# paperwave/STIF-continuous-video-representation

Measured on AMD Instinct MI355X. Metric: upsampled Mpix/sec at 7×128×128→4× scale, 1/2/4/8 MI355X; PSNR vs ref, higher is better.
Workload: dtype f16x3; 1 GPU; per GPU 7x3x128x128 window (6 pairs), 4.0x spatial, t=[0.5]; frames=7, parallelism=1 GPU

## Files before the change

stif-continuous-video-representation_amd/csrc/decoder.hip:

```cpp
#include "dec_layout.h"
#include "stif_common.h"
#include "tuning.h"
#include "stif.h"
#include "abi_util.h"

#include <algorithm>
#include <climits>
#include <cstdio>
#include <type_traits>

namespace {

using namespace stif_dec;

template <int F16>
struct XT;
template <>
struct XT<0> {
  f32x16 v;
};
template <>
struct XT<1> {
  f16x8 h[2], l[2];
};
// ... 73 lines not shown
  b.w00 = (vx0 && vy0) ? wx0 * wy0 : 0.f;
  b.w01 = (vx1 && vy0) ? wx1 * wy0 : 0.f;
  b.w10 = (vx0 && vy1) ? wx0 * wy1 : 0.f;
  b.w11 = (vx1 && vy1) ? wx1 * wy1 : 0.f;
  return b;
}
STIF_DEV Bilin bilin(float gx, float gy, int Wd, int Hd) {
  const Corners c = bilin_corners(gx, gy, Wd, Hd);
  Bilin b;
  b.o00 = c.cy0 * Wd + c.cx0; b.o01 = c.cy0 * Wd + c.cx1; b.o10 = c.cy1 * Wd + c.cx0; b.o11 = c.cy1 * Wd + c.cx1;
  b.w00 = c.w00; b.w01 = c.w01; b.w10 = c.w10; b.w11 = c.w11;
  return b;
}

template <class TAB>
STIF_DEV Bilin bilin_tab(const TAB& tb, int py, int px, int pitch) {
  Bilin b;
  const int *by0 = tb.by0, *by1 = tb.by1, *bx0 = tb.bx0, *bx1 = tb.bx1;
  const float *wy0_ = tb.wy0, *wy1_ = tb.wy1, *wx0_ = tb.wx0, *wx1_ = tb.wx1;
  const int y0 = by0[py], y1 = by1[py], x0 = bx0[px], x1 = bx1[px];
  const float wy0 = wy0_[py], wy1 = wy1_[py], wx0 = wx0_[px], wx1 = wx1_[px];
  b.o00 = y0 * pitch + x0; b.o01 = y0 * pitch + x1; b.o10 = y1 * pitch + x0; b.o11 = y1 * pitch + x1;
  b.w00 = wx0 * wy0; b.w01 = wx1 * wy0; b.w10 = wx0 * wy1; b.w11 = wx1 * wy1;
  return b;
}

struct WarpGrids {
  float g1x, g1y, g2x, g2y;
};
STIF_DEV WarpGrids warp_grids(const f32x4 fv, float bx, float by, int WW, int HH) {
  const float lo = -1.f + 1e-6f, hi = 1.f - 1e-6f;
  const float dx = ((float)WW - 1.f) / 2.f, dy = ((float)HH - 1.f) / 2.f;
  WarpGrids g;
  g.g1x = fminf(fmaxf(bx + fv[0] / dx, lo), hi), g.g1y = fminf(fmaxf(by + fv[1] / dy, lo), hi);
  g.g2x = fminf(fmaxf(bx + fv[2] / dx, lo), hi), g.g2y = fminf(fmaxf(by + fv[3] / dy, lo), hi);
  return g;
}

constexpr int GRID = 0, WINDOW = 1, PTS = 2;

template <bool OR>
STIF_DEV void report_range_w(int* status, bool bad) {
  if constexpr (OR) {
    if (status != nullptr && bad) atomicOr(status, 1);
  } else {
    report_range(status, bad);
  }
}

template <int FORM>
STIF_DEV Bilin bilin_hr(float gx, float gy, int WW, int HH, const stif_dec_window& win, int* status, int slot = 0) {
  if constexpr (FORM == GRID) {
    return bilin(gx, gy, WW, HH);
  } else if constexpr (FORM == PTS) {
    const Corners c = bilin_corners(gx, gy, WW, HH);
    Bilin b;
    b.o00 = slot; b.o01 = slot + 1; b.o10 = slot + 2; b.o11 = slot + 3;
    b.w00 = c.w00; b.w01 = c.w01; b.w10 = c.w10; b.w11 = c.w11;
    return b;
  } else {
    const Corners c = bilin_corners(gx, gy, WW, HH);
    const int ry0 = c.cy0 - win.fy0, ry1 = c.cy1 - win.fy0, rx0 = c.cx0 - win.fx0, rx1 = c.cx1 - win.fx0;
    const int y0 = min(max(ry0, 0), win.fh - 1), y1 = min(max(ry1, 0), win.fh - 1);
    const int x0 = min(max(rx0, 0), win.fw - 1), x1 = min(max(rx1, 0), win.fw - 1);
    if (status != nullptr && (y0 != ry0 || y1 != ry1 || x0 != rx0 || x1 != rx1)) atomicOr(status, 2);
    Bilin b;
    b.o00 = y0 * win.fw + x0; b.o01 = y0 * win.fw + x1; b.o10 = y1 * win.fw + x0; b.o11 = y1 * win.fw + x1;
    b.w00 = c.w00; b.w01 = c.w01; b.w10 = c.w10; b.w11 = c.w11;
    return b;
  }
}

template <int GPB>
STIF_DEV void gather64(f32x16* dst, const float* __restrict__ base, int stride, int c0, const Bilin& b, int hf) {
  const int c = c0 + 4 * hf;
  const float* p00 = base + (size_t)b.o00 * stride + c;
  const float* p01 = base + (size_t)b.o01 * stride + c;
  const float* p10 = base + (size_t)b.o10 * stride + c;
  const float* p11 = base + (size_t)b.o11 * stride + c;
#pragma unroll
  for (int g0 = 0; g0 < 8; g0 += GPB) {
    f32x4 cr[GPB][4];
#pragma unroll
    for (int g = 0; g < GPB; ++g) {
      const int o = 8 * (g0 + g);
      cr[g][0] = ld4(p00 + o);
      cr[g][1] = ld4(p01 + o);
      cr[g][2] = ld4(p10 + o);
      cr[g][3] = ld4(p11 + o);
    }
#pragma unroll
    for (int g = 0; g < GPB; ++g) {
      f32x4 s = b.w00 * cr[g][0] + b.w01 * cr[g][1] + b.w10 * cr[g][2] + b.w11 * cr[g][3];
      asm volatile("" : "+v"(s));
      const int gg = g0 + g;
#pragma unroll
      for (int e = 0; e < 4; ++e) dst[gg >> 2][4 * (gg & 3) + e] = s[e];
    }
    if constexpr (GPB < 8) asm volatile("" ::: "memory");
  }
}

STIF_DEV void img_mma(f32x16* z, const float* __restrict__ wt, const f32x4 im4, int lane) {
#pragma unroll
  for (int ot = 0; ot < 2; ++ot) {
    const f32x4 w0 = ld4(wt + ot * T + lane * 4);
#pragma unroll
    for (int e = 0; e < 4; ++e) z[ot] = mfma32(w0[e], im4[e], z[ot]);
  }
}

STIF_DEV f32x4 img_sample(const float* __restrict__ I, const Bilin& b, int hf) {
  const float* c = I + 4 * hf;
  return b.w00 * ld4(c + b.o00 * IMG_C) + b.w01 * ld4(c + b.o01 * IMG_C) + b.w10 * ld4(c + b.o10 * IMG_C) +
         b.w11 * ld4(c + b.o11 * IMG_C);
}

struct Pixel {
  bool valid;
  long long pc;
  int item, ly, lx;
  int pt;
};
STIF_DEV void point_yx(const stif_dec_points& pts, int item, int pt, int HH, int WW, int* status, int& y, int& x) {
  const int ry = pts.y[item * pts.y_item + pt], rx = pts.x[item * pts.x_item + pt];
  y = min(max(ry, 0), HH - 1), x = min(max(rx, 0), WW - 1);
  if (status != nullptr && (y != ry || x != rx)) atomicOr(status, 8);
}
template <int NW, int PPW, int FORM, class TQ>
STIF_DEV Pixel pixel_of(int wv, int lane, int n, int HH, int WW, const stif_dec_window& win, const TQ& tq,
                        int* status) {
  Pixel o;
  if constexpr (FORM == PTS) {
    const long long total = (long long)n * tq.npts;
    const long long p = ((long long)xcd_block(blockIdx.x, gridDim.x) * NW + wv) * PPW + (lane & (PPW - 1));
    o.valid = p < total;
    o.pc = o.valid ? p : total - 1;
    o.item = (int)(o.pc / tq.npts);
    o.pt = (int)(o.pc - (long long)o.item * tq.npts);
    point_yx(tq, o.item, o.pt, HH, WW, status, o.ly, o.lx);
  } else {
    constexpr bool WIN = FORM == WINDOW;
    const int GH = WIN ? win.hh : HH, GW = WIN ? win.ww : WW;
    const long long total = (long long)n * GH * GW;
    const long long p = ((long long)xcd_block(blockIdx.x, gridDim.x) * NW + wv) * PPW + (lane & (PPW - 1));
    o.valid = p < total;
    o.pc = o.valid ? p : total - 1;
    o.item = (int)(o.pc / ((long long)GH * GW));
    const int rem = (int)(o.pc - (long long)o.item * GH * GW);
    o.ly = rem / GW, o.lx = rem - o.ly * GW;
    o.pt = 0;
  }
  return o;
}

template <int TQ>
struct TimeArg {
  typedef const float* __restrict__ type;
};
template <>
struct TimeArg<1> {
  typedef stif_dec_time type;
};
template <>
struct TimeArg<2> {
  typedef stif_dec_points type;
};
template <int FORM, bool TF>
constexpr int TQK = FORM == PTS ? 2 : TF ? 1 : 0;
template <int TQ>
STIF_DEV float time_at(const typename TimeArg<TQ>::type& tq, int item, int gy, int gx, int pt = 0) {
  if constexpr (TQ == 2) return tq.t[item * tq.t_item + pt * tq.t_point];
  else if constexpr (TQ == 1) return tq.t[item * tq.item + gy * tq.row + gx * tq.col];
  else return tq[item];
}

STIF_DEV float blend_weight(const stif_dec_blend& bl, int gy, int gx) {
#pragma clang fp contract(off)
  float a[4];
#pragma unroll
  for (int j = 0; j < 4; ++j) a[j] = __fadd_rn(fabsf(__fmul_rn(bl.rel_y[j][gy], bl.rel_x[j][gx])), 1e-9f);
  const float tot = __fadd_rn(__fadd_rn(__fadd_rn(a[0], a[1]), a[2]), a[3]);
  const float ak = bl.k == 0 ? a[3] : bl.k == 1 ? a[2] : bl.k == 2 ? a[1] : a[0];
  return __fdiv_rn(ak, tot);
}

template <int FORM, bool REPORT, bool BLEND = false>
STIF_DEV void store_rgb(float* __restrict__ out, const float* __restrict__ mlp, const float* o4, const f32x4 fv,
                        int item, int py, int px, int HH, int WW, const stif_dec_window& win, int* status,
                        const stif_dec_blend& bl) {
  constexpr bool WIN = FORM == WINDOW;
  static_assert(WIN || !BLEND, "the blending epilogue is the windowed stages'");
  const size_t plane = WIN ? (size_t)win.out_plane : (size_t)HH * WW;
  float* o = WIN ? out + (size_t)item * win.out_item + (size_t)py * win.out_pitch + px
                 : out + (size_t)item * 3 * plane + (size_t)py * WW + px;
  bool bad = not_finite((fv[0] + fv[1]) + (fv[2] + fv[3]));
  float rgb[3];
#pragma unroll
  for (int c = 0; c < 3; ++c) {
    rgb[c] = o4[c] + mlp[E_B4 + c];
    bad |= not_finite(rgb[c]);
    if constexpr (!BLEND) o[c * plane] = rgb[c];
  }
  if constexpr (BLEND) {
    const float wk = blend_weight(bl, win.y0 + py, win.x0 + px);
    if (!bl.accumulate) {
#pragma unroll
      for (int c = 0; c < 3; ++c) o[c * plane] = __fmul_rn(rgb[c], wk);
    } else {
#pragma unroll
      for (int c = 0; c < 3; ++c) o[c * plane] = __fmaf_rn(rgb[c], wk, o[c * plane]);
    }
  }
  if constexpr (REPORT) report_range_w<FORM != GRID>(status, bad);
}

constexpr int NW1 = 4;
constexpr int DEC2_NW = 4;
constexpr int DEC2_WPE = 2;
constexpr int SEG = 10;
constexpr int SEG1 = 8;

STIF_DEV void dec_dma(__amdgpu_buffer_rsrc_t rm, float* dst, int lane, int soff) {
  __builtin_amdgcn_raw_ptr_buffer_load_lds(rm, dst, 16, (unsigned)(lane * 16), soff, 0, 0);
}
template <int NW>
STIF_DEV void dma_tiles(float* dst, __amdgpu_buffer_rsrc_t rm, int src, int ntiles, int wv, int lane) {
  if ((ntiles * 4) % NW == 0) {
#pragma unroll
    for (int i = 0; i < ntiles * 4 / NW; ++i)
      dec_dma(rm, dst + (wv + i * NW) * 256, lane, (src + (wv + i * NW) * 256) * 4);
  } else {
    for (int k = wv; k < ntiles * 4; k += NW)
      dec_dma(rm, dst + k * 256, lane, (src + k * 256) * 4);
  }
}

STIF_DEV __amdgpu_buffer_rsrc_t mlp_rsrc(const float* mlp) {
  return __builtin_amdgcn_make_buffer_rsrc((void*)mlp, (short)0, (int)(MLP_FLOATS * 4), 0x00020000);
}

template <int F16>
STIF_DEV void tile_mma(f32x16& acc, const float* t, const XT<F16>& xt, int lane) {
  const float* b = t + lane * 4;
  if constexpr (F16) {
#pragma unroll
    for (int m = 0; m < 2; ++m) {
      const f16x8 ah = ldh8(b + (2 * m) * 256), al = ldh8(b + (2 * m + 1) * 256);
      acc = mfma16h(ah, xt.h[m], acc);
      acc = mfma16h(al, xt.h[m], acc);
      acc = mfma16h(ah, xt.l[m], acc);
    }
  } else {
    const f32x16& x = xt.v;
    const f32x4 w0 = ld4(b), w1 = ld4(b + 256), w2 = ld4(b + 512), w3 = ld4(b + 768);
#pragma unroll
    for (int e = 0; e < 4; ++e) acc = mfma32(w0[e], x[e], acc);
#pragma unroll
    for (int e = 0; e < 4; ++e) acc = mfma32(w1[e], x[4 + e], acc);
#pragma unroll
    for (int e = 0; e < 4; ++e) acc = mfma32(w2[e], x[8 + e], acc);
#pragma unroll
    for (int e = 0; e < 4; ++e) acc = mfma32(w3[e], x[12 + e], acc);
  }
  __builtin_amdgcn_sched_barrier(0);
}

template <int NO>
STIF_DEV void narrow_dot(float* o, const float* W, int kt, const f32x16& x, int hf) {
#pragma unroll
  for (int c = 0; c < NO; ++c)
#pragma unroll
    for (int v = 0; v < 4; ++v) {
      const f32x4 w = ld4(W + c * 256 + kt * 32 + 8 * v + 4 * hf);
#pragma unroll
      for (int e = 0; e < 4; ++e) o[c] = fmaf(w[e], x[4 * v + e], o[c]);
    }
}

template <int MODE, bool HRIMG>
constexpr int OCC1 = MODE == 2 ? 2 : HRIMG ? 3 : 4;
template <int MODE, bool HRIMG>
constexpr int S1 = OCC1<MODE, HRIMG> == 4 ? 4 : OCC1<MODE, HRIMG> == 3 ? 6 : SEG1;
template <int MODE, bool HRIMG, int F16, int FORM, bool TF = false>
__global__ __launch_bounds__(NW1 * 64) __attribute__((amdgpu_waves_per_eu(OCC1<MODE, HRIMG>))) void k_dec1(const float* __restrict__ proj, const float* __restrict__ mlp,
                                                     stif_dec_tables tb, stif_dec_image im,
                                                     typename TimeArg<TQK<FORM, TF>>::type tq, float* __restrict__ hrfeat,
                                                     float* __restrict__ flow, int n, int h, int w, int HH,
                                                     int WW, stif_dec_window win, int* status) {
  constexpr bool WIN = FORM == WINDOW;
  constexpr int TQ = TQK<FORM, TF>;
  static_assert(!(WIN && MODE == 2 && HRIMG), "the windowed flow-only stage takes no high-resolution image");
  static_assert(!TF || (MODE != 2 && !HRIMG), "a time field has no local-ensemble and no HR-image form");
  static_assert(FORM != PTS || (MODE != 2 && !HRIMG && !TF), "a point list has no local-ensemble and no HR-image form");
  constexpr bool OCC3 = S1<MODE, HRIMG> != SEG1;
  constexpr bool OCC4 = OCC1<MODE, HRIMG> == 4;
  __shared__ __attribute__((aligned(16))) float wbuf[2 * S1<MODE, HRIMG> * T + T];
  const int lane = threadIdx.x & 63, hf = lane >> 5;
  const int wv = __builtin_amdgcn_readfirstlane(threadIdx.x >> 6);
  float* const B0 = wbuf;
  float* const B1 = wbuf + S1<MODE, HRIMG> * T;
  float* const W3V = wbuf + 2 * S1<MODE, HRIMG> * T;
  const __amdgpu_buffer_rsrc_t rm = mlp_rsrc(mlp);
  if (MODE != 1) dma_tiles<NW1>(W3V, rm, L_W3V, 1, wv, lane);
  if (MODE != 2) dma_tiles<NW1>(B0, rm, F_W1, 4, wv, lane);
  else {
    dma_tiles<NW1>(B1, rm, L_W0, 4, wv, lane);
    dma_tiles<NW1>(B1 + 4 * T, rm, L_W1, 4, wv, lane);
  }
  const Pixel pix = pixel_of<NW1, 32, FORM>(wv, lane, n, HH, WW, win, tq, status);
  const bool valid = pix.valid;
  const long long pc = pix.pc;
  const int item = pix.item;
  const int py = WIN ? win.y0 + pix.ly : pix.ly, px = WIN ? win.x0 + pix.lx : pix.lx;
  const float t = TF ? 0.f : time_at<TQ>(tq, item, py, px, pix.pt);
  auto time = [&]() {
    if constexpr (TF) return time_at<TQ>(tq, item, py, px);
    else return t;
  };
  const float* P = proj + (size_t)item * h * w * PROJ_C;

  f32x16 hr[2] = {f32x16{0}, f32x16{0}};
  f32x16 x1[2];
  if constexpr (MODE != 2) {
  f32x16 x0[2];
  {
    const float ry = tb.rel_y[py], rx = tb.rel_x[px], t = time();
    const float* p1 = P + ((size_t)tb.near_y[py] * w + tb.near_x[px]) * PROJ_C;
#pragma unroll
    for (int ot = 0; ot < 2; ++ot)
#pragma unroll
      for (int v = 0; v < 4; ++v) {
        const int f = ot * 32 + 8 * v + 4 * hf;
        const f32x4 z = ld4(p1 + f) + ld4(mlp + F_WRY + f) * ry + ld4(mlp + F_WRX + f) * rx + ld4(mlp + F_WT + f) * t;
#pragma unroll
        for (int e = 0; e < 4; ++e) x0[ot][4 * v + e] = siren_sin<F16>(z[e]);
      }
  }
  auto seg_feat23 = [&](float* dst, int kt) {
#pragma unroll
    for (int r = 0; r < 16 / NW1; ++r) {
      const int i = wv + r * NW1, j = i >> 2;
      const int src = (j < 2 ? F_W2 + (kt * 2 + j) * T : F_W3 + ((j - 2) * 8 + kt) * T) + (i & 3) * 256;
      dec_dma(rm, dst + j * T + (i & 3) * 256, lane, src * 4);
    }
  };
  lds_dma_barrier();
  const Bias32 fb1[2] = {bias_ld(mlp + F_B1, hf), bias_ld(mlp + F_B1 + 32, hf)};
  __builtin_amdgcn_sched_barrier(0);
  seg_feat23(B1, 0);
  {
    const XT<F16> xs[2] = {xop<F16>(x0[0]), xop<F16>(x0[1])};
#pragma unroll
    for (int ot = 0; ot < 2; ++ot) {
      f32x16 acc = f32x16{0};
#pragma unroll
      for (int kt = 0; kt < 2; ++kt) tile_mma<F16>(acc, B0 + (ot * 2 + kt) * T, xs[kt], lane);
      x1[ot] = bias_sin<F16>(acc, fb1[ot]);
    }
  }
  const XT<F16> x1s[2] = {xop<F16>(x1[0]), xop<F16>(x1[1])};
  auto feat_step = [&](int kt, bool last) {
    lds_dma_barrier();
    const Bias32 b2 = bias_ld(mlp + F_B2 + kt * 32, hf);
    __builtin_amdgcn_sched_barrier(0);
    float* cur = (kt & 1) ? B0 : B1;
    float* nxt = (kt & 1) ? B1 : B0;
    if (!last) seg_feat23(nxt, kt + 1);
    else {
      dma_tiles<NW1>(nxt, rm, L_W0, 4, wv, lane);
      if (!OCC4) dma_tiles<NW1>(nxt + 4 * T, rm, L_W1, OCC3 ? 2 : 4, wv, lane);
    }
    f32x16 acc = f32x16{0};
    tile_mma<F16>(acc, cur, x1s[0], lane);
    tile_mma<F16>(acc, cur + T, x1s[1], lane);
    const XT<F16> h2 = xop<F16>(bias_sin<F16>(acc, b2));
    tile_mma<F16>(hr[0], cur + 2 * T, h2, lane);
    tile_mma<F16>(hr[1], cur + 3 * T, h2, lane);
  };
#pragma unroll 1
  for (int kt = 0; kt < 7; ++kt) feat_step(kt, false);
  feat_step(7, true);
#pragma unroll
  for (int ot = 0; ot < 2; ++ot) hr[ot] = bias_add<F16>(hr[ot], mlp + F_B3 + ot * 32, hf);
  if (valid) {
    float* o = hrfeat + (WIN ? ((size_t)item * win.fh + (py - win.fy0)) * win.fw + (px - win.fx0) : (size_t)pc) * 64;
#pragma unroll
    for (int ot = 0; ot < 2; ++ot)
#pragma unroll
      for (int v = 0; v < 4; ++v) {
        f32x4 s;
#pragma unroll
        for (int e = 0; e < 4; ++e) s[e] = hr[ot][4 * v + e];
        st4(o + ot * 32 + 8 * v + 4 * hf, s);
      }
  }
  }
  if constexpr (MODE == 1) return;
  if constexpr (MODE == 2) {
    Bilin b;
    if constexpr (WIN) {
      const int ry = tb.hr_y[py] - win.fy0, rx = tb.hr_x[px] - win.fx0;
      const int y = min(max(ry, 0), win.fh - 1), x = min(max(rx, 0), win.fw - 1);
      if (status != nullptr && (y != ry || x != rx)) atomicOr(status, 4);
      b.o00 = b.o01 = b.o10 = b.o11 = y * win.fw + x;
    } else {
      b.o00 = b.o01 = b.o10 = b.o11 = tb.hr_y[py] * WW + tb.hr_x[px];
    }
    b.w00 = 1.f;
    b.w01 = b.w10 = b.w11 = 0.f;
    gather64<8>(hr, hrfeat + (size_t)item * (WIN ? (size_t)win.fh * win.fw : (size_t)HH * WW) * 64, 64, 0, b, hf);
  }

  f32x16 z[2];
  {
    const Bilin b = bilin_tab(tb, py, px, w);
    const float t = time();
    if (OCC4) gather64<2>(z, P, PROJ_C, 64, b, hf);
    else if (OCC3) gather64<4>(z, P, PROJ_C, 64, b, hf);
    else gather64<8>(z, P, PROJ_C, 64, b, hf);
#pragma unroll
    for (int ot = 0; ot < 2; ++ot)
#pragma unroll
      for (int v = 0; v < 4; ++v) {
        const int f = ot * 32 + 8 * v + 4 * hf;
        const f32x4 wt = ld4(mlp + L_WT + f), bb = ld4(mlp + L_B0 + f);
#pragma unroll
        for (int e = 0; e < 4; ++e) z[ot][4 * v + e] = (z[ot][4 * v + e] + (wt[e] * t + bb[e])) * ACC_IN<F16>;
      }
    if constexpr (HRIMG) {
      const Bilin bi = bilin_tab(im, py, px, im.iw);
      img_mma(z, mlp + I_L, img_sample(im.img + (size_t)item * im.ih * im.iw * IMG_C, bi, hf), lane);
    }
  }
  lds_dma_barrier();
  const Bias32 lb1[2] = {bias_ld(mlp + L_B1, hf), bias_ld(mlp + L_B1 + 32, hf)};
  __builtin_amdgcn_sched_barrier(0);
  auto seg_flow23 = [&](float* dst, int kt) {
    dma_tiles<NW1>(dst, rm, L_W2 + kt * 2 * T, 2, wv, lane);
  };
  constexpr bool L1B0 = OCC3 && !OCC4 && MODE == 0;
  if (OCC4) dma_tiles<NW1>(B0, rm, L_W1, 4, wv, lane);
  else {
    if (L1B0) dma_tiles<NW1>(B0, rm, L_W1 + 2 * T, 2, wv, lane);
    seg_flow23(B0 + (L1B0 ? 2 * T : 0), 0);
  }
  {
    const XT<F16> hs[2] = {xop<F16>(hr[0]), xop<F16>(hr[1])};
#pragma unroll
    for (int ot = 0; ot < 2; ++ot) {
#pragma unroll
      for (int kt = 0; kt < 2; ++kt) tile_mma<F16>(z[ot], B1 + (ot * 2 + kt) * T, hs[kt], lane);
#pragma unroll
      for (int r = 0; r < 16; ++r) z[ot][r] = siren_sin<F16>(z[ot][r] * ACC_S<F16>);
    }
  }
  if (L1B0 || OCC4) lds_dma_barrier();
  if (OCC4) seg_flow23(B1, 0);
  {
    const XT<F16> zs[2] = {xop<F16>(z[0]), xop<F16>(z[1])};
#pragma unroll
    for (int ot = 0; ot < 2; ++ot) {
      f32x16 acc = f32x16{0};
      const float* w1t = OCC4 ? B0 + ot * 2 * T : (L1B0 && ot == 1) ? B0 : B1 + (4 + ot * 2) * T;
#pragma unroll
      for (int kt = 0; kt < 2; ++kt) tile_mma<F16>(acc, w1t + kt * T, zs[kt], lane);
      x1[ot] = bias_sin<F16>(acc, lb1[ot]);
    }
  }
  const XT<F16> x1f[2] = {xop<F16>(x1[0]), xop<F16>(x1[1])};
  float fl[4] = {0.f, 0.f, 0.f, 0.f};
  auto flow_step = [&](int kt, bool last) {
    lds_dma_barrier();
    const Bias32 b2 = bias_ld(mlp + L_B2 + kt * 32, hf);
    __builtin_amdgcn_sched_barrier(0);
    float* cur = OCC4 ? ((kt & 1) ? B0 : B1) : (kt & 1) ? B1 : (L1B0 && kt == 0 ? B0 + 2 * T : B0);
    float* nxt = OCC4 ? ((kt & 1) ? B1 : B0) : (kt & 1) ? B0 : B1;
    if (!last) seg_flow23(nxt, kt + 1);
    f32x16 acc = f32x16{0};
    tile_mma<F16>(acc, cur, x1f[0], lane);
    tile_mma<F16>(acc, cur + T, x1f[1], lane);
    const f32x16 h2 = bias_sin<F16>(acc, b2);
    narrow_dot<4>(fl, W3V, kt, h2, hf);
  };
#pragma unroll 1
  for (int kt = 0; kt < 7; ++kt) flow_step(kt, false);
  flow_step(7, true);
#pragma unroll
  for (int c = 0; c < 4; ++c) fl[c] += __shfl_xor(fl[c], 32);
  if (valid && hf == 0) {
    const f32x4 bb = ld4(mlp + L_B3);
    f32x4 s;
#pragma unroll
    for (int e = 0; e < 4; ++e) s[e] = fl[e] + bb[e];
    st4(flow + (size_t)pc * 4, s);
  }
}

template <bool HRIMG, int F16, int FORM, bool BLEND = false, bool TF = false>
__global__ __launch_bounds__(DEC2_NW * 64) __attribute__((amdgpu_waves_per_eu(DEC2_WPE))) void k_dec2(const float* __restrict__ proj, const float* __restrict__ mlp,
                                                     const float* __restrict__ hrfeat, const float* __restrict__ flow,
                                                     stif_dec_tables tb, stif_dec_image im,
                                                     typename TimeArg<TQK<FORM, TF>>::type tq, float* __restrict__ out, int n,
                                                     int h, int w, int HH, int WW, int* status, stif_dec_window win,
                                                     stif_dec_blend bl) {
  constexpr bool WIN = FORM == WINDOW;
  constexpr int TQ = TQK<FORM, TF>;
  static_assert(!TF || (!HRIMG && !BLEND), "a time field has no HR-image and no blending form");
  static_assert(FORM != PTS || (!HRIMG && !BLEND && !TF), "a point list has no HR-image and no blending form");
  __shared__ __attribute__((aligned(16))) float wbuf[2 * SEG * T];
  const int lane = threadIdx.x & 63, hf = lane >> 5;
  const int wv = __builtin_amdgcn_readfirstlane(threadIdx.x >> 6);
  float* const B0 = wbuf;
  float* const B1 = wbuf + SEG * T;
  const __amdgpu_buffer_rsrc_t rm = mlp_rsrc(mlp);
  dma_tiles<DEC2_NW>(B0, rm, E_W0, 8, wv, lane);
  const Pixel pix = pixel_of<DEC2_NW, 32, FORM>(wv, lane, n, HH, WW, win, tq, status);
  const long long pc = pix.pc;
  const int item = pix.item, py = pix.ly, px = pix.lx;
  const float t = time_at<TQ>(tq, item, WIN ? win.y0 + py : py, WIN ? win.x0 + px : px, pix.pt);
  const float* P = proj + (size_t)item * h * w * PROJ_C;
  const float* HRF = hrfeat + (WIN ? (size_t)item * win.fh * win.fw * 64 : (size_t)item * HH * WW * 64);
  if constexpr (FORM == PTS) HRF = hrfeat + (size_t)item * tq.npts * 8 * 64;

  const f32x4 fv = ld4(flow + (size_t)pc * 4);
  const float bx = tb.lin_x[WIN ? win.x0 + px : px], by = tb.lin_y[WIN ? win.y0 + py : py];
  const WarpGrids wg = warp_grids(fv, bx, by, WW, HH);

  f32x16 x0[2];
  {
    f32x16 z[2], q[2];
    gather64<8>(z, P, PROJ_C, 128, bilin(wg.g1x, wg.g1y, w, h), hf);
    asm volatile("" ::: "memory");
    gather64<8>(q, P, PROJ_C, 192, bilin(wg.g2x, wg.g2y, w, h), hf);
#pragma unroll
    for (int ot = 0; ot < 2; ++ot)
#pragma unroll
      for (int v = 0; v < 4; ++v) {
        const int f = ot * 32 + 8 * v + 4 * hf;
        const f32x4 wt = ld4(mlp + E_WT + f), bb = ld4(mlp + E_B0 + f);
#pragma unroll
        for (int e = 0; e < 4; ++e) z[ot][4 * v + e] = (z[ot][4 * v + e] + (q[ot][4 * v + e] + wt[e] * t + bb[e])) * ACC_IN<F16>;
      }
    if constexpr (HRIMG) {
      const float* I = im.img + (size_t)item * im.ih * im.iw * IMG_C;
      img_mma(z, mlp + I_E1, img_sample(I, bilin(wg.g1x, wg.g1y, im.iw, im.ih), hf), lane);
      img_mma(z, mlp + I_E2, img_sample(I, bilin(wg.g2x, wg.g2y, im.iw, im.ih), hf), lane);
    }
    asm volatile("" ::: "memory");
    gather64<8>(q, HRF, 64, 0, bilin_hr<FORM>(wg.g1x, wg.g1y, WW, HH, win, status, 8 * pix.pt), hf);
    lds_dma_barrier();
    dma_tiles<DEC2_NW>(B1, rm, E_W1, 4, wv, lane);
    {
      const XT<F16> qs[2] = {xop<F16>(q[0]), xop<F16>(q[1])};
#pragma unroll
      for (int ot = 0; ot < 2; ++ot)
#pragma unroll
        for (int kt = 0; kt < 2; ++kt) tile_mma<F16>(z[ot], B0 + (ot * 4 + kt) * T, qs[kt], lane);
    }
    asm volatile("" ::: "memory");
    gather64<8>(q, HRF, 64, 0, bilin_hr<FORM>(wg.g2x, wg.g2y, WW, HH, win, status, 8 * pix.pt + 4), hf);
    const XT<F16> qs[2] = {xop<F16>(q[0]), xop<F16>(q[1])};
#pragma unroll
    for (int ot = 0; ot < 2; ++ot) {
#pragma unroll
      for (int kt = 2; kt < 4; ++kt) tile_mma<F16>(z[ot], B0 + (ot * 4 + kt) * T, qs[kt - 2], lane);
#pragma unroll
      for (int r = 0; r < 16; ++r) x0[ot][r] = siren_sin<F16>(z[ot][r] * ACC_S<F16>);
    }
  }
  lds_dma_barrier();
  const Bias32 eb1[2] = {bias_ld(mlp + E_B1, hf), bias_ld(mlp + E_B1 + 32, hf)};
  __builtin_amdgcn_sched_barrier(0);
  auto seg_l23 = [&](float* dst, int kt) {
    dma_tiles<DEC2_NW>(dst, rm, E_W2 + kt * 2 * T, 2, wv, lane);
#pragma unroll
    for (int ot = 0; ot < 8; ++ot) dma_tiles<DEC2_NW>(dst + (2 + ot) * T, rm, E_W3 + (ot * 8 + kt) * T, 1, wv, lane);
  };
  seg_l23(B0, 0);
  f32x16 x1[2];
  {
    const XT<F16> xs[2] = {xop<F16>(x0[0]), xop<F16>(x0[1])};
#pragma unroll
    for (int ot = 0; ot < 2; ++ot) {
      f32x16 acc = f32x16{0};
#pragma unroll
      for (int kt = 0; kt < 2; ++kt) tile_mma<F16>(acc, B1 + (ot * 2 + kt) * T, xs[kt], lane);
      x1[ot] = bias_sin<F16>(acc, eb1[ot]);
    }
  }
  const XT<F16> x1s[2] = {xop<F16>(x1[0]), xop<F16>(x1[1])};
  f32x16 a3[8];
#pragma unroll
  for (int ot = 0; ot < 8; ++ot) a3[ot] = f32x16{0};
  auto l23_step = [&](int kt, bool last) {
    lds_dma_barrier();
    const Bias32 b2 = bias_ld(mlp + E_B2 + kt * 32, hf);
    __builtin_amdgcn_sched_barrier(0);
    float* cur = (kt & 1) ? B1 : B0;
    float* nxt = (kt & 1) ? B0 : B1;
    if (!last) seg_l23(nxt, kt + 1);
    else dma_tiles<DEC2_NW>(nxt, rm, E_W4V, 1, wv, lane);
    f32x16 acc = f32x16{0};
    tile_mma<F16>(acc, cur, x1s[0], lane);
    tile_mma<F16>(acc, cur + T, x1s[1], lane);
    const XT<F16> h2 = xop<F16>(bias_sin<F16>(acc, b2));
#pragma unroll
    for (int ot = 0; ot < 8; ++ot) tile_mma<F16>(a3[ot], cur + (2 + ot) * T, h2, lane);
  };
#pragma unroll 1
  for (int kt = 0; kt < 7; ++kt) l23_step(kt, false);
  l23_step(7, true);
  lds_dma_barrier();
  float o4[3] = {0.f, 0.f, 0.f};
#pragma unroll
  for (int kt = 0; kt < 8; ++kt) {
    const f32x16 h3 = bias_sin<F16>(a3[kt], B0 + (E_W4V_B3 - E_W4V) + kt * 32, hf);
    narrow_dot<3>(o4, B0, kt, h3, hf);
  }
#pragma unroll
  for (int c = 0; c < 3; ++c) o4[c] += __shfl_xor(o4[c], 32);
  if (pix.valid && hf == 0) {
    if constexpr (FORM == PTS) store_rgb<PTS, F16 != 0>(out, mlp, o4, fv, item, 0, pix.pt, 1, tq.npts, win, status, bl);
    else store_rgb<FORM, F16 != 0, BLEND>(out, mlp, o4, fv, item, py, px, HH, WW, win, status, bl);
  }
}


constexpr int DEC2Q_NW = 8;
constexpr int SEGQ = 10;
static_assert(SEGQ * 4 % DEC2Q_NW == 0, "k_dec2q: every wave issues the same number of LDS-DMA pieces");
static_assert(2 * SEGQ * T * 4 * 2 <= 160 * 1024, "k_dec2q: two workgroups per CU, their LDS within 160 KB");
struct R32 {
  f32x4 s[2];
};
struct XQ {
  f16x8 h, l;
};
STIF_DEV XQ xq(const R32& x) {
  XQ o;
  split_f16x3(x.s[0], x.s[1], o.h, o.l);
  return o;
}
STIF_DEV void tile_q(R32& acc, const float* t, const XQ& x, int lane) {
  const float* b = t + lane * 4;
#pragma unroll
  for (int s = 0; s < 2; ++s) {
    const f16x8 ah = ldh8(b + (2 * s) * 256), al = ldh8(b + (2 * s + 1) * 256);
    acc.s[s] = __builtin_amdgcn_mfma_f32_16x16x32_f16(ah, x.h, acc.s[s], 0, 0, 0);
    acc.s[s] = __builtin_amdgcn_mfma_f32_16x16x32_f16(al, x.h, acc.s[s], 0, 0, 0);
    acc.s[s] = __builtin_amdgcn_mfma_f32_16x16x32_f16(ah, x.l, acc.s[s], 0, 0, 0);
  }
  __builtin_amdgcn_sched_barrier(0);
}
STIF_DEV R32 bias_q(const float* __restrict__ b, int q) {
  R32 o;
#pragma unroll
  for (int s = 0; s < 2; ++s) o.s[s] = ld4(b + 16 * s + 4 * q);
  return o;
}
STIF_DEV R32 bias_sin_q(const R32& z, const R32& bb) {
  R32 o;
#pragma unroll
  for (int s = 0; s < 2; ++s)
#pragma unroll
    for (int e = 0; e < 4; ++e) o.s[s][e] = siren_sin<1>(fmaf(z.s[s][e], ACC_S<1>, bb.s[s][e]));
  return o;
}
STIF_DEV R32 bias_sin_q(const R32& z, const float* __restrict__ b, int q) { return bias_sin_q(z, bias_q(b, q)); }
STIF_DEV void gather_q(R32* dst, const float* __restrict__ base, int stride, int c0, const Bilin& b, int q) {
  const int c = c0 + 4 * q;
  const float* p00 = base + (size_t)b.o00 * stride + c;
  const float* p01 = base + (size_t)b.o01 * stride + c;
  const float* p10 = base + (size_t)b.o10 * stride + c;
  const float* p11 = base + (size_t)b.o11 * stride + c;
  f32x4 cr[4][4];
#pragma unroll
  for (int g = 0; g < 4; ++g) {
    cr[g][0] = ld4(p00 + 16 * g);
    cr[g][1] = ld4(p01 + 16 * g);
    cr[g][2] = ld4(p10 + 16 * g);
    cr[g][3] = ld4(p11 + 16 * g);
  }
#pragma unroll
  for (int g = 0; g < 4; ++g) {
    f32x4 v = b.w00 * cr[g][0] + b.w01 * cr[g][1] + b.w10 * cr[g][2] + b.w11 * cr[g][3];
    asm volatile("" : "+v"(v));
    dst[g >> 1].s[g & 1] = v;
  }
}

template <int FORM, bool BLEND = false, bool TF = false>
__global__ __launch_bounds__(DEC2Q_NW * 64) __attribute__((amdgpu_waves_per_eu(4))) void k_dec2q(
    const float* __restrict__ proj, const float* __restrict__ mlp, const float* __restrict__ hrfeat,
    const float* __restrict__ flow, stif_dec_tables tb, typename TimeArg<TQK<FORM, TF>>::type tq,
    float* __restrict__ out, int n, int h, int w, int HH, int WW, int* status, stif_dec_window win, stif_dec_blend bl) {
  constexpr bool WIN = FORM == WINDOW;
  constexpr int TQ = TQK<FORM, TF>;
  static_assert(!TF || !BLEND, "a time field has no blending form");
  static_assert(FORM != PTS || (!BLEND && !TF), "a point list has no blending form");
  __shared__ __attribute__((aligned(16))) float wbuf[2 * SEGQ * T];
  const int lane = threadIdx.x & 63, q = lane >> 4;
  const int wv = __builtin_amdgcn_readfirstlane(threadIdx.x >> 6);
  constexpr int NW = DEC2Q_NW;
  float* const B0 = wbuf;
  float* const B1 = wbuf + SEGQ * T;
  const __amdgpu_buffer_rsrc_t rm = mlp_rsrc(mlp);
  dma_tiles<NW>(B0, rm, Q_W0, 8, wv, lane);
  auto seg_l23 = [&](float* dst, int kt) {
#pragma unroll
    for (int r = 0; r < SEGQ * 4 / NW; ++r) {
      const int i = wv + r * NW;
      const int j = i >> 2;
      const int src = (j < 2 ? Q_W2 + (kt * 2 + j) * T : Q_W3 + ((j - 2) * 8 + kt) * T) + (i & 3) * 256;
      dec_dma(rm, dst + j * T + (i & 3) * 256, lane, src * 4);
    }
  };
  const Pixel pix = pixel_of<NW, 16, FORM>(wv, lane, n, HH, WW, win, tq, status);
  const long long pc = pix.pc;
  const int item = pix.item, py = pix.ly, px = pix.lx;
  const float t = time_at<TQ>(tq, item, WIN ? win.y0 + py : py, WIN ? win.x0 + px : px, pix.pt);
  const float* P = proj + (size_t)item * h * w * PROJ_C;
  const float* HRF = hrfeat + (WIN ? (size_t)item * win.fh * win.fw * 64 : (size_t)item * HH * WW * 64);
  if constexpr (FORM == PTS) HRF = hrfeat + (size_t)item * tq.npts * 8 * 64;

  const f32x4 fv = ld4(flow + (size_t)pc * 4);
  const float bx = tb.lin_x[WIN ? win.x0 + px : px], by = tb.lin_y[WIN ? win.y0 + py : py];
  const WarpGrids wg = warp_grids(fv, bx, by, WW, HH);

  R32 x0[2];
  {
    R32 z[2], g[2];
    gather_q(z, P, PROJ_C, 128, bilin(wg.g1x, wg.g1y, w, h), q);
    asm volatile("" ::: "memory");
    gather_q(g, P, PROJ_C, 192, bilin(wg.g2x, wg.g2y, w, h), q);
#pragma unroll
    for (int ot = 0; ot < 2; ++ot)
#pragma unroll
      for (int s = 0; s < 2; ++s) {
        const int f = 32 * ot + 16 * s + 4 * q;
        const f32x4 wt = ld4(mlp + E_WT + f), bb = ld4(mlp + E_B0 + f);
#pragma unroll
        for (int e = 0; e < 4; ++e)
          z[ot].s[s][e] = (z[ot].s[s][e] + (g[ot].s[s][e] + wt[e] * t + bb[e])) * ACC_IN<1>;
      }
    asm volatile("" ::: "memory");
    gather_q(g, HRF, 64, 0, bilin_hr<FORM>(wg.g1x, wg.g1y, WW, HH, win, status, 8 * pix.pt), q);
    lds_dma_barrier();
    dma_tiles<NW>(B1, rm, Q_W1, 4, wv, lane);
    {
      const XQ qs[2] = {xq(g[0]), xq(g[1])};
#pragma unroll
      for (int ot = 0; ot < 2; ++ot)
#pragma unroll
        for (int kt = 0; kt < 2; ++kt) tile_q(z[ot], B0 + (ot * 4 + kt) * T, qs[kt], lane);
    }
    asm volatile("" ::: "memory");
    gather_q(g, HRF, 64, 0, bilin_hr<FORM>(wg.g2x, wg.g2y, WW, HH, win, status, 8 * pix.pt + 4), q);
    const XQ qs[2] = {xq(g[0]), xq(g[1])};
#pragma unroll
    for (int ot = 0; ot < 2; ++ot) {
#pragma unroll
      for (int kt = 2; kt < 4; ++kt) tile_q(z[ot], B0 + (ot * 4 + kt) * T, qs[kt - 2], lane);
#pragma unroll
      for (int s = 0; s < 2; ++s)
#pragma unroll
        for (int e = 0; e < 4; ++e) x0[ot].s[s][e] = siren_sin<1>(z[ot].s[s][e] * ACC_S<1>);
    }
  }
  lds_dma_barrier();
  const R32 eb1[2] = {bias_q(mlp + E_B1, q), bias_q(mlp + E_B1 + 32, q)};
  __builtin_amdgcn_sched_barrier(0);
  seg_l23(B0, 0);
  R32 x1[2];
  {
    const XQ xs[2] = {xq(x0[0]), xq(x0[1])};
#pragma unroll
    for (int ot = 0; ot < 2; ++ot) {
      R32 acc;
      acc.s[0] = acc.s[1] = f32x4{0.f, 0.f, 0.f, 0.f};
#pragma unroll
      for (int kt = 0; kt < 2; ++kt) tile_q(acc, B1 + (ot * 2 + kt) * T, xs[kt], lane);
      x1[ot] = bias_sin_q(acc, eb1[ot]);
    }
  }
  const XQ x1s[2] = {xq(x1[0]), xq(x1[1])};
  R32 a3[8];
#pragma unroll
  for (int ot = 0; ot < 8; ++ot) a3[ot].s[0] = a3[ot].s[1] = f32x4{0.f, 0.f, 0.f, 0.f};
  auto l23_step = [&](int kt, bool last) {
    lds_dma_barrier();
    const R32 b2 = bias_q(mlp + E_B2 + kt * 32, q);
    __builtin_amdgcn_sched_barrier(0);
    float* cur = (kt & 1) ? B1 : B0;
    float* nxt = (kt & 1) ? B0 : B1;
    if (!last) seg_l23(nxt, kt + 1);
    else dma_tiles<NW>(nxt, rm, E_W4V, 1, wv, lane);
    R32 acc;
    acc.s[0] = acc.s[1] = f32x4{0.f, 0.f, 0.f, 0.f};
    tile_q(acc, cur, x1s[0], lane);
    tile_q(acc, cur + T, x1s[1], lane);
    const XQ h2 = xq(bias_sin_q(acc, b2));
#pragma unroll
    for (int ot = 0; ot < 8; ++ot) tile_q(a3[ot], cur + (2 + ot) * T, h2, lane);
  };
#pragma unroll 1
  for (int kt = 0; kt < 7; ++kt) l23_step(kt, false);
  l23_step(7, true);
  lds_dma_barrier();
  float o4[3] = {0.f, 0.f, 0.f};
#pragma unroll
  for (int kt = 0; kt < 8; ++kt) {
    const R32 h3 = bias_sin_q(a3[kt], B0 + (E_W4V_B3 - E_W4V) + kt * 32, q);
#pragma unroll
    for (int c = 0; c < 3; ++c)
#pragma unroll
      for (int s = 0; s < 2; ++s) {
        const f32x4 wr = ld4(B0 + c * 256 + kt * 32 + 16 * s + 4 * q);
#pragma unroll
        for (int e = 0; e < 4; ++e) o4[c] = fmaf(wr[e], h3.s[s][e], o4[c]);
      }
  }
#pragma unroll
  for (int c = 0; c < 3; ++c) {
    o4[c] += __shfl_xor(o4[c], 16);
    o4[c] += __shfl_xor(o4[c], 32);
  }
  if (pix.valid && q == 0) {
    if constexpr (FORM == PTS) store_rgb<PTS, true>(out, mlp, o4, fv, item, 0, pix.pt, 1, tq.npts, win, status, bl);
    else store_rgb<FORM, true, BLEND>(out, mlp, o4, fv, item, py, px, HH, WW, win, status, bl);
  }
}

__global__ void k_dec_bounds_init(int* __restrict__ box) {
  if (threadIdx.x < 4) box[threadIdx.x] = (threadIdx.x & 1) ? INT_MIN : INT_MAX;
}
__global__ __launch_bounds__(256) void k_dec_bounds(const float* __restrict__ flow, stif_dec_tables tb,
                                                    int* __restrict__ box, long long total, int HH, int WW,
                                                    stif_dec_window win) {
  int ymin = INT_MAX, ymax = INT_MIN, xmin = INT_MAX, xmax = INT_MIN;
  const int plane = win.hh * win.ww;
  for (long long p = (long long)blockIdx.x * 256 + threadIdx.x; p < total; p += (long long)gridDim.x * 256) {
    const int rem = (int)(p % plane);
    const int py = rem / win.ww, px = rem - py * win.ww;
    const WarpGrids g = warp_grids(ld4(flow + (size_t)p * 4), tb.lin_x[win.x0 + px], tb.lin_y[win.y0 + py], WW, HH);
    const Corners a = bilin_corners(g.g1x, g.g1y, WW, HH), b = bilin_corners(g.g2x, g.g2y, WW, HH);
    ymin = min(ymin, min(min(a.cy0, a.cy1), min(b.cy0, b.cy1)));
    ymax = max(ymax, max(max(a.cy0, a.cy1), max(b.cy0, b.cy1)));
    xmin = min(xmin, min(min(a.cx0, a.cx1), min(b.cx0, b.cx1)));
    xmax = max(xmax, max(max(a.cx0, a.cx1), max(b.cx0, b.cx1)));
  }
#pragma unroll
  for (int m = 32; m >= 1; m >>= 1) {
    ymin = min(ymin, __shfl_xor(ymin, m));
    ymax = max(ymax, __shfl_xor(ymax, m));
    xmin = min(xmin, __shfl_xor(xmin, m));
    xmax = max(xmax, __shfl_xor(xmax, m));
  }
  if ((threadIdx.x & 63) == 0 && ymin <= ymax) {
    atomicMin(box + 0, ymin);
    atomicMax(box + 1, ymax);
    atomicMin(box + 2, xmin);
    atomicMax(box + 3, xmax);
  }
}

__global__ __launch_bounds__(256) void k_dec_corners(const float* __restrict__ flow, stif_dec_tables tb,
                                                     stif_dec_points pts, int* __restrict__ cy, int* __restrict__ cx,
                                                     float* __restrict__ ct, long long total, int HH, int WW,
                                                     int* status) {
  for (long long p = (long long)blockIdx.x * 256 + threadIdx.x; p < total; p += (long long)gridDim.x * 256) {
    const int item = (int)(p / pts.npts), pt = (int)(p - (long long)item * pts.npts);
    int y, x;
    point_yx(pts, item, pt, HH, WW, status, y, x);
    const float t = time_at<2>(pts, item, y, x, pt);
    const WarpGrids g = warp_grids(ld4(flow + (size_t)p * 4), tb.lin_x[x], tb.lin_y[y], WW, HH);
    const Corners c[2] = {bilin_corners(g.g1x, g.g1y, WW, HH), bilin_corners(g.g2x, g.g2y, WW, HH)};
#pragma unroll
    for (int k = 0; k < 8; ++k) {
      const Corners& a = c[k >> 2];
      cy[p * 8 + k] = (k & 2) ? a.cy1 : a.cy0;
      cx[p * 8 + k] = (k & 1) ? a.cx1 : a.cx0;
      ct[p * 8 + k] = t;
    }
  }
}

__global__ __launch_bounds__(256) void k_pack_lr(const float* __restrict__ f0, const float* __restrict__ f1,
                                                 const float* __restrict__ f2, const float* __restrict__ x,
                                                 float* __restrict__ out, int n, int h, int w) {
  const long long npix = (long long)n * h * w;
  for (long long e = (long long)blockIdx.x * 256 + threadIdx.x; e < npix * 50; e += (long long)gridDim.x * 256) {
    const long long pix = e / 50;
    const int q = (int)(e - pix * 50);
    f32x4 v;
    if (q < 48) {
      const float* src = q < 16 ? f0 : (q < 32 ? f1 : f2);
      v = ld4(src + pix * 64 + (q & 15) * 4);
    } else {
      const int item = (int)(pix / ((long long)h * w));
      const long long yx = pix - (long long)item * h * w;
      const float* xi = x + (size_t)item * 6 * h * w + yx;
      const size_t pl = (size_t)h * w;
      if (q == 48) { v[0] = xi[0]; v[1] = xi[pl]; v[2] = xi[2 * pl]; v[3] = xi[3 * pl]; }
      else { v[0] = xi[4 * pl]; v[1] = xi[5 * pl]; v[2] = 0.f; v[3] = 0.f; }
    }
    st4(out + pix * SRC_C + q * 4, v);
  }
}

__global__ __launch_bounds__(256) void k_blend4(const float* __restrict__ p0, const float* __restrict__ p1,
// ... 427 lines not shown
```

Before: 101.7 Mpix/s.

## Coalesce decoder bilinear gathers via DPP broadcast and LDS transpose, stash pixel coords

In the quad decoder kernel, each bilinear gather now broadcasts one pixel's four corner addresses across a 16-lane row with DPP. Each row then reads a whole contiguous 64-channel record, and the blended values are transposed back to the owning lanes through a per-wave swizzled LDS block. This replaces scattered per-lane 16-byte loads with coalesced 256-byte reads, at the cost of extra LDS traffic, wave barriers and a lane permutation of the warp grids. In the first decoder kernel, pixel indices are stashed in LDS or recomputed late so they do not stay live in registers across the MLP loops, lowering register pressure to keep four workgroups per CU.

```diff
diff --git a/stif-continuous-video-representation_amd/csrc/decoder.hip b/stif-continuous-video-representation_amd/csrc/decoder.hip
--- a/stif-continuous-video-representation_amd/csrc/decoder.hip
+++ b/stif-continuous-video-representation_amd/csrc/decoder.hip
@@ -249,6 +249,18 @@
     o.pt = 0;
   }
   return o;
+}
+
+template <int NW, int PPW, int FORM, class TQ>
+STIF_DEV void pixel_slot(int wv, int lane, int n, int HH, int WW, const stif_dec_window& win, const TQ& tq, bool& valid,
+                         long long& pc) {
+  asm volatile("" : "+v"(lane));
+  long long total;
+  if constexpr (FORM == PTS) total = (long long)n * tq.npts;
+  else total = (long long)n * (FORM == WINDOW ? win.hh : HH) * (FORM == WINDOW ? win.ww : WW);
+  const long long p = ((long long)xcd_block(blockIdx.x, gridDim.x) * NW + wv) * PPW + (lane & (PPW - 1));
+  valid = p < total;
+  pc = valid ? p : total - 1;
 }
 
 template <int TQ>
@@ -406,8 +418,6 @@
     dma_tiles<NW1>(B1 + 4 * T, rm, L_W1, 4, wv, lane);
   }
   const Pixel pix = pixel_of<NW1, 32, FORM>(wv, lane, n, HH, WW, win, tq, status);
-  const bool valid = pix.valid;
-  const long long pc = pix.pc;
   const int item = pix.item;
   const int py = WIN ? win.y0 + pix.ly : pix.ly, px = WIN ? win.x0 + pix.lx : pix.lx;
   const float t = TF ? 0.f : time_at<TQ>(tq, item, py, px, pix.pt);
@@ -416,6 +426,22 @@
     else return t;
   };
   const float* P = proj + (size_t)item * h * w * PROJ_C;
+  constexpr bool STASH = OCC4 && (MODE == 0 || WIN);
+  __shared__ int stash[STASH ? 3 * NW1 * 64 : 1];
+  static_assert(!STASH || 4 * (sizeof(wbuf) + sizeof(stash)) <= 160 * 1024, "k_dec1: four workgroups per CU, their LDS within 160 KB");
+  if constexpr (STASH) {
+    stash[threadIdx.x] = item;
+    stash[NW1 * 64 + threadIdx.x] = py;
+    stash[2 * NW1 * 64 + threadIdx.x] = px;
+  }
+  auto pixel_again = [&](int& ai, int& ay, int& ax) {
+    if constexpr (STASH) {
+      ai = stash[threadIdx.x], ay = stash[NW1 * 64 + threadIdx.x], ax = stash[2 * NW1 * 64 + threadIdx.x];
+    } else {
+      ai = item, ay = py, ax = px;
+      asm volatile("" : "+v"(ai), "+v"(ay), "+v"(ax));
+    }
+  };
 
   f32x16 hr[2] = {f32x16{0}, f32x16{0}};
   f32x16 x1[2];
@@ -480,8 +506,16 @@
   feat_step(7, true);
 #pragma unroll
   for (int ot = 0; ot < 2; ++ot) hr[ot] = bias_add<F16>(hr[ot], mlp + F_B3 + ot * 32, hf);
+  bool valid;
+  long long pc;
+  pixel_slot<NW1, 32, FORM>(wv, lane, n, HH, WW, win, tq, valid, pc);
   if (valid) {
-    float* o = hrfeat + (WIN ? ((size_t)item * win.fh + (py - win.fy0)) * win.fw + (px - win.fx0) : (size_t)pc) * 64;
+    float* o = hrfeat + (size_t)pc * 64;
+    if constexpr (WIN) {
+      int si, sy, sx;
+      pixel_again(si, sy, sx);
+      o = hrfeat + (((size_t)si * win.fh + (sy - win.fy0)) * win.fw + (sx - win.fx0)) * 64;
+    }
 #pragma unroll
     for (int ot = 0; ot < 2; ++ot)
 #pragma unroll
@@ -511,7 +545,10 @@
 
   f32x16 z[2];
   {
-    const Bilin b = bilin_tab(tb, py, px, w);
+    int fi, fy, fx;
+    pixel_again(fi, fy, fx);
+    const float* P = proj + (size_t)fi * h * w * PROJ_C;
+    const Bilin b = bilin_tab(tb, fy, fx, w);
     const float t = time();
     if (OCC4) gather64<2>(z, P, PROJ_C, 64, b, hf);
     else if (OCC3) gather64<4>(z, P, PROJ_C, 64, b, hf);
@@ -526,8 +563,8 @@
         for (int e = 0; e < 4; ++e) z[ot][4 * v + e] = (z[ot][4 * v + e] + (wt[e] * t + bb[e])) * ACC_IN<F16>;
       }
     if constexpr (HRIMG) {
-      const Bilin bi = bilin_tab(im, py, px, im.iw);
-      img_mma(z, mlp + I_L, img_sample(im.img + (size_t)item * im.ih * im.iw * IMG_C, bi, hf), lane);
+      const Bilin bi = bilin_tab(im, fy, fx, im.iw);
+      img_mma(z, mlp + I_L, img_sample(im.img + (size_t)fi * im.ih * im.iw * IMG_C, bi, hf), lane);
     }
   }
   lds_dma_barrier();
@@ -585,6 +622,9 @@
   flow_step(7, true);
 #pragma unroll
   for (int c = 0; c < 4; ++c) fl[c] += __shfl_xor(fl[c], 32);
+  bool valid;
+  long long pc;
+  pixel_slot<NW1, 32, FORM>(wv, lane, n, HH, WW, win, tq, valid, pc);
   if (valid && hf == 0) {
     const f32x4 bb = ld4(mlp + L_B3);
     f32x4 s;
@@ -765,26 +805,59 @@
   return o;
 }
 STIF_DEV R32 bias_sin_q(const R32& z, const float* __restrict__ b, int q) { return bias_sin_q(z, bias_q(b, q)); }
-STIF_DEV void gather_q(R32* dst, const float* __restrict__ base, int stride, int c0, const Bilin& b, int q) {
-  const int c = c0 + 4 * q;
-  const float* p00 = base + (size_t)b.o00 * stride + c;
-  const float* p01 = base + (size_t)b.o01 * stride + c;
-  const float* p10 = base + (size_t)b.o10 * stride + c;
-  const float* p11 = base + (size_t)b.o11 * stride + c;
+template <int N>
+STIF_DEV int row_bcast(int v) {
+  return __builtin_amdgcn_mov_dpp(v, 0x150 + N, 0xf, 0xf, false);
+}
+template <int N>
+STIF_DEV float row_bcast(float v) {
+  return __builtin_bit_cast(float, row_bcast<N>(__builtin_bit_cast(int, v)));
+}
+template <int N>
+STIF_DEV unsigned long long row_bcast(unsigned long long a) {
+  const unsigned lo = (unsigned)row_bcast<N>((int)(unsigned)a), hi = (unsigned)row_bcast<N>((int)(unsigned)(a >> 32));
+  return ((unsigned long long)hi << 32) | lo;
+}
+STIF_DEV int fetch_of(int v, int lane) {
+  return __builtin_amdgcn_ds_bpermute(((lane & 48) | ((lane + (lane >> 4)) & 15)) * 4, v);
+}
+STIF_DEV float fetch_of(float v, int lane) {
+  return __builtin_bit_cast(float, fetch_of(__builtin_bit_cast(int, v), lane));
+}
+template <int G>
+STIF_DEV void fetch_q(f32x4* cr, const unsigned long long* rec, int lane) {
+  typedef const f32x4 __attribute__((address_space(1)))* gptr4;
+#pragma unroll
+  for (int c = 0; c < 4; ++c) cr[c] = *(gptr4)(row_bcast<4 * G>(rec[c]) + 16 * (lane & 15));
+}
+template <int G>
+STIF_DEV void blend_q(float* blk, const f32x4* cr, const Bilin& b, int lane) {
+  const float w00 = row_bcast<4 * G>(b.w00), w01 = row_bcast<4 * G>(b.w01), w10 = row_bcast<4 * G>(b.w10),
+              w11 = row_bcast<4 * G>(b.w11);
+  f32x4 v = w00 * cr[0] + w01 * cr[1] + w10 * cr[2] + w11 * cr[3];
+  asm volatile("" : "+v"(v));
+  const int r = lane >> 4, j = lane & 15;
+  st4(blk + (4 * G + r) * 64 + (((j ^ r) * 4) ^ (16 * G)), v);
+}
+STIF_DEV void gather_q(R32* dst, const float* __restrict__ base, int stride, int c0, const Bilin& b, float* blk,
+                       int lane) {
+  const unsigned long long rec[4] = {
+      (unsigned long long)(base + (size_t)b.o00 * stride + c0), (unsigned long long)(base + (size_t)b.o01 * stride + c0),
+      (unsigned long long)(base + (size_t)b.o10 * stride + c0), (unsigned long long)(base + (size_t)b.o11 * stride + c0)};
   f32x4 cr[4][4];
-#pragma unroll
-  for (int g = 0; g < 4; ++g) {
-    cr[g][0] = ld4(p00 + 16 * g);
-    cr[g][1] = ld4(p01 + 16 * g);
-    cr[g][2] = ld4(p10 + 16 * g);
-    cr[g][3] = ld4(p11 + 16 * g);
-  }
-#pragma unroll
-  for (int g = 0; g < 4; ++g) {
-    f32x4 v = b.w00 * cr[g][0] + b.w01 * cr[g][1] + b.w10 * cr[g][2] + b.w11 * cr[g][3];
-    asm volatile("" : "+v"(v));
-    dst[g >> 1].s[g & 1] = v;
-  }
+  fetch_q<0>(cr[0], rec, lane);
+  fetch_q<1>(cr[1], rec, lane);
+  fetch_q<2>(cr[2], rec, lane);
+  fetch_q<3>(cr[3], rec, lane);
+  blend_q<0>(blk, cr[0], b, lane);
+  blend_q<1>(blk, cr[1], b, lane);
+  blend_q<2>(blk, cr[2], b, lane);
+  blend_q<3>(blk, cr[3], b, lane);
+  __builtin_amdgcn_wave_barrier();
+  const int p = lane & 15, q = lane >> 4;
+#pragma unroll
+  for (int g = 0; g < 4; ++g) dst[g >> 1].s[g & 1] = ld4(blk + p * 64 + (((q ^ p) * 4) ^ (16 * g)));
+  __builtin_amdgcn_wave_barrier();
 }
 
 template <int FORM, bool BLEND = false, bool TF = false>
@@ -817,20 +890,25 @@
   const long long pc = pix.pc;
   const int item = pix.item, py = pix.ly, px = pix.lx;
   const float t = time_at<TQ>(tq, item, WIN ? win.y0 + py : py, WIN ? win.x0 + px : px, pix.pt);
-  const float* P = proj + (size_t)item * h * w * PROJ_C;
-  const float* HRF = hrfeat + (WIN ? (size_t)item * win.fh * win.fw * 64 : (size_t)item * HH * WW * 64);
-  if constexpr (FORM == PTS) HRF = hrfeat + (size_t)item * tq.npts * 8 * 64;
 
   const f32x4 fv = ld4(flow + (size_t)pc * 4);
   const float bx = tb.lin_x[WIN ? win.x0 + px : px], by = tb.lin_y[WIN ? win.y0 + py : py];
-  const WarpGrids wg = warp_grids(fv, bx, by, WW, HH);
+  WarpGrids wg = warp_grids(fv, bx, by, WW, HH);
+  wg.g1x = fetch_of(wg.g1x, lane), wg.g1y = fetch_of(wg.g1y, lane);
+  wg.g2x = fetch_of(wg.g2x, lane), wg.g2y = fetch_of(wg.g2y, lane);
+  const int fitem = fetch_of(item, lane), fpt = FORM == PTS ? fetch_of(pix.pt, lane) : 0;
+  const float* P = proj + (size_t)fitem * h * w * PROJ_C;
+  const float* HRF = hrfeat + (WIN ? (size_t)fitem * win.fh * win.fw * 64 : (size_t)fitem * HH * WW * 64);
+  if constexpr (FORM == PTS) HRF = hrfeat + (size_t)fitem * tq.npts * 8 * 64;
+  static_assert(NW == 8 && SEGQ == 10, "k_dec2q: the gathers' LDS blocks are tiles 4..9 of B1 and 8, 9 of B0");
+  float* const blk = wv < 6 ? B1 + (4 + wv) * T : B0 + (2 + wv) * T;
 
   R32 x0[2];
   {
     R32 z[2], g[2];
-    gather_q(z, P, PROJ_C, 128, bilin(wg.g1x, wg.g1y, w, h), q);
+    gather_q(z, P, PROJ_C, 128, bilin(wg.g1x, wg.g1y, w, h), blk, lane);
     asm volatile("" ::: "memory");
-    gather_q(g, P, PROJ_C, 192, bilin(wg.g2x, wg.g2y, w, h), q);
+    gather_q(g, P, PROJ_C, 192, bilin(wg.g2x, wg.g2y, w, h), blk, lane);
 #pragma unroll
     for (int ot = 0; ot < 2; ++ot)
 #pragma unroll
@@ -842,7 +920,7 @@
           z[ot].s[s][e] = (z[ot].s[s][e] + (g[ot].s[s][e] + wt[e] * t + bb[e])) * ACC_IN<1>;
       }
     asm volatile("" ::: "memory");
-    gather_q(g, HRF, 64, 0, bilin_hr<FORM>(wg.g1x, wg.g1y, WW, HH, win, status, 8 * pix.pt), q);
+    gather_q(g, HRF, 64, 0, bilin_hr<FORM>(wg.g1x, wg.g1y, WW, HH, win, status, 8 * fpt), blk, lane);
     lds_dma_barrier();
     dma_tiles<NW>(B1, rm, Q_W1, 4, wv, lane);
     {
@@ -853,7 +931,7 @@
         for (int kt = 0; kt < 2; ++kt) tile_q(z[ot], B0 + (ot * 4 + kt) * T, qs[kt], lane);
     }
     asm volatile("" ::: "memory");
-    gather_q(g, HRF, 64, 0, bilin_hr<FORM>(wg.g2x, wg.g2y, WW, HH, win, status, 8 * pix.pt + 4), q);
+    gather_q(g, HRF, 64, 0, bilin_hr<FORM>(wg.g2x, wg.g2y, WW, HH, win, status, 8 * fpt + 4), blk, lane);
     const XQ qs[2] = {xq(g[0]), xq(g[1])};
 #pragma unroll
     for (int ot = 0; ot < 2; ++ot) {
```

Result: no change. 102.4 Mpix/s, median of 6 (+0.8%).
